# Jutho/Strided.jl

Hardware: AMD Instinct MI355X
Metric: GB/s effective HBM for @strided permutedims!+broadcast, 32^4 fp64 (higher is better)
Workload: dtype f64; 1 GPU; configs[1]+configs[2]: permutedims!(B,A,(4,3,2,1)) then C .= sum of 4 permuted views of A, 32x32x32x32 Float64, one set of arrays (A, B, C) per GPU.  C is a THIRD array chosen so that the two statements share only the read-only A and overlap; the README writes both into B -- that form is `step_same_destination` on the --full line; parallelism=replicas x1 (independent arrays per rank)

## Files before the change

include/strided_hip.h:

```cpp
#ifndef STRIDED_HIP_H
#define STRIDED_HIP_H

#include <stddef.h>
#include <stdint.h>

#ifdef __cplusplus
extern "C" {
#endif

#define SMR_ABI_VERSION 1
#define SMR_MAXN 8
#define SMR_MAXM 8
#define SMR_MAXPROG 96
#define SMR_MAXCONST 16

typedef enum {
    SMR_OK = 0,
    SMR_EINVAL = -1,
    SMR_EUNSUPPORTED = -2,
    SMR_EHIP = -3,
    SMR_ENOMEM = -4,
    SMR_ENODEVICE = -5
} smr_status;

// ... 106 lines not shown
    int64_t strides[SMR_MAXN];
    int32_t dtype;
    int32_t conj;
} smr_operand;

typedef struct smr_problem {
    int32_t N;
    int32_t M;
    int64_t dims[SMR_MAXN];
    smr_operand ops[SMR_MAXM];
    const uint8_t* fprog;
    int32_t fprog_len;
    int32_t nconsts;
    const double* fconsts;
    int32_t redop;
    int32_t initop;
    double initarg[2];
    void* stream;
} smr_problem;

typedef struct smr_plan smr_plan;

int smr_abi_version(void);
int smr_init(int device);
int smr_shutdown(void);
int smr_device_count(void);
const char* smr_last_error(void);
int smr_malloc(size_t bytes, void** out);
int smr_free(void* p);
int smr_memcpy_h2d(void* dst, const void* src, size_t bytes, void* stream);
int smr_memcpy_d2h(void* dst, const void* src, size_t bytes, void* stream);
int smr_stream_sync(void* stream);

int smr_overlap_begin(void* stream);
int smr_overlap_end(void* stream);
int smr_overlap_fence(void* stream);
int smr_stream_create(void** out);
int smr_stream_destroy(void* stream);

typedef struct smr_seq smr_seq;
int smr_seq_create(smr_seq** out);
int smr_seq_add(smr_seq* seq, smr_plan* plan, void* const* bases);
int smr_seq_run(smr_seq* seq, int reps, void* stream);
int smr_seq_wait(smr_seq* seq);
int smr_seq_info(smr_seq* seq, char* buf, size_t buflen);
int smr_seq_components(smr_seq* seq, int32_t* comp, size_t cap);
int smr_seq_fences(smr_seq* seq, int32_t* acquire, size_t cap, int64_t* footprint, int32_t* cache_resident);
int smr_seq_set(smr_seq* seq, const char* name, int64_t value);
int smr_seq_destroy(smr_seq* seq);
int smr_debug_kernarg_layout(const void* elf, size_t bytes, const char* symbol, int index, int32_t* out, char* name_out, size_t name_cap);
int smr_debug_canon_prog(const smr_problem* problem, uint8_t* code, int cap, int* nwraps, int* compute_class, int32_t* orig);
int smr_debug_seq_schedule(int nexec, const int32_t* nspans, const int64_t* spans, const int32_t* launches, const int64_t* knobs, const int32_t* comp_slices,
                           int32_t* per_exec, int32_t* totals, int64_t* footprint, int32_t* packets, int packet_cap);


int smr_mapreduce(const smr_problem* problem);
int smr_mapreduce_scalar(const smr_problem* problem, void* host_result);

int smr_plan_create(const smr_problem* problem, smr_plan** out);
int smr_plan_execute(smr_plan* plan, void* const* bases, void* stream);
int smr_plan_destroy(smr_plan* plan);
int smr_plan_prepare(smr_plan* plan);
int smr_plan_describe(const smr_plan* plan, char* buf, size_t buflen);
int64_t smr_plan_algorithmic_bytes(const smr_plan* plan);
int64_t smr_plan_tile_order(const smr_plan* plan, uint32_t* out, size_t cap);
int64_t smr_plan_orbit_pairs(const smr_plan* plan, uint32_t* out, size_t cap);
int64_t smr_plan_flat_runs(const smr_plan* plan, int64_t* out, size_t cap);
int64_t smr_plan_flat_side(const smr_plan* plan, int64_t* out, size_t cap);
int64_t smr_plan_flat_batched(const smr_plan* plan, int64_t* out, size_t cap);

int smr_plan_jit_compile(smr_plan* plan, size_t* code_size);
int smr_plan_jit_source(const smr_plan* plan, char* buf, size_t buflen);

int smr_shard(const smr_problem* problem, int nshards, int shard, smr_problem* out,
              int* needs_allreduce);
int smr_shard_ex(const smr_problem* problem, int nshards, int shard, uint32_t local_ops,
                 smr_problem* out, int* needs_allreduce, int* split_dim, int64_t* start,
                 int64_t* stop);
int smr_init_reduction(const smr_problem* problem);

int smr_comm_unique_id(void* out, size_t len);
int smr_comm_init(int nranks, int rank, const void* unique_id, size_t len);
int smr_comm_rank(int* rank, int* nranks);
int smr_comm_library(char* buf, size_t buflen);
int smr_comm_destroy(void);
int smr_mapreduce_sharded(const smr_problem* problem);
int smr_mapreduce_sharded_ex(const smr_problem* problem, uint32_t local_ops);

int smr_set_option(const char* name, int64_t value);
int64_t smr_get_option(const char* name);

#ifdef __cplusplus
}
#endif
#endif
```

strided.jl_amd/_lib.py:

```python
from __future__ import annotations

import ctypes as C
import os
import subprocess

SMR_MAXN = 8
SMR_MAXM = 8
SMR_MAXPROG = 96
SMR_MAXCONST = 16

SMR_OK, SMR_EINVAL, SMR_EUNSUPPORTED, SMR_EHIP, SMR_ENOMEM, SMR_ENODEVICE = 0, -1, -2, -3, -4, -5

(SMR_F32, SMR_F64, SMR_C32, SMR_C64, SMR_I8, SMR_I16, SMR_I32, SMR_I64,
 SMR_U8, SMR_U16, SMR_U32, SMR_U64, SMR_BOOL) = range(13)

SMR_RED_NONE, SMR_RED_ADD, SMR_RED_MUL, SMR_RED_MIN, SMR_RED_MAX, SMR_RED_AND, SMR_RED_OR = range(7)
(SMR_INIT_NONE, SMR_INIT_IDENTITY, SMR_INIT_ZERO, SMR_INIT_SCALE, SMR_INIT_CONST,
 SMR_INIT_CONJ) = range(6)

OPCODES = dict(
    ARG=0, CONST=1,
    NEG=8, ABS=9, ABS2=10, CONJ=11, REAL=12, IMAG=13, SQRT=14, EXP=15, LOG=16, SIN=17, COS=18,
    TANH=19, INV=20, ROUND32=21, WIDEN=22,
    ADD=32, SUB=33, MUL=34, DIV=35, MIN=36, MAX=37, LT=38, LE=39, GT=40, GE=41, EQ=42, NE=43,
    SELECT=64, FMA=65,
    POWI=96, TAN=97, ASIN=98, ACOS=99, ATAN=100, SINH=101, COSH=102, EXP2=103, EXPM1=104, LOG2=105, LOG10=106, LOG1P=107,
    CBRT=108, FLOOR=109, CEIL=110, TRUNC=111, ROUND=112, SIGN=113, NOT=114,
    POW=128, ATAN2=129, HYPOT=130, REM=131, MOD=132, AND=133, OR=134, XOR=135,
)


class smr_operand(C.Structure):
    _fields_ = [
        ("base", C.c_void_p),
        ("offset", C.c_int64),
        ("strides", C.c_int64 * SMR_MAXN),
        ("dtype", C.c_int32),
        ("conj", C.c_int32),
    ]


class smr_problem(C.Structure):
    _fields_ = [
        ("N", C.c_int32),
        ("M", C.c_int32),
        ("dims", C.c_int64 * SMR_MAXN),
        ("ops", smr_operand * SMR_MAXM),
        ("fprog", C.POINTER(C.c_uint8)),
        ("fprog_len", C.c_int32),
        ("nconsts", C.c_int32),
        ("fconsts", C.POINTER(C.c_double)),
        ("redop", C.c_int32),
        ("initop", C.c_int32),
        ("initarg", C.c_double * 2),
        ("stream", C.c_void_p),
    ]


_PKG_DIR = os.path.dirname(os.path.abspath(__file__))
LIB_PATH = os.environ.get("SMR_LIB") or os.path.join(_PKG_DIR, "libstrided_hip.so")
CSRC_DIR = os.path.join(_PKG_DIR, "csrc")

EXPORTS = [
    "smr_abi_version", "smr_init", "smr_shutdown", "smr_device_count", "smr_last_error",
    "smr_malloc", "smr_free", "smr_memcpy_h2d", "smr_memcpy_d2h", "smr_stream_sync",
    "smr_mapreduce", "smr_plan_create", "smr_plan_execute", "smr_plan_destroy",
    "smr_plan_describe", "smr_plan_algorithmic_bytes", "smr_plan_tile_order", "smr_plan_orbit_pairs", "smr_plan_flat_runs", "smr_plan_flat_side", "smr_plan_flat_batched", "smr_mapreduce_scalar", "smr_plan_jit_compile", "smr_plan_jit_source", "smr_plan_prepare", "smr_comm_unique_id", "smr_comm_init", "smr_comm_rank", "smr_comm_library",
    "smr_comm_destroy", "smr_mapreduce_sharded", "smr_mapreduce_sharded_ex", "smr_shard", "smr_shard_ex", "smr_init_reduction", "smr_set_option",
    "smr_get_option", "smr_overlap_begin", "smr_overlap_end", "smr_overlap_fence", "smr_stream_create", "smr_stream_destroy",
    "smr_seq_create", "smr_seq_add", "smr_seq_run", "smr_seq_wait", "smr_seq_info", "smr_seq_components", "smr_seq_fences", "smr_seq_set", "smr_seq_destroy", "smr_debug_kernarg_layout", "smr_debug_canon_prog", "smr_debug_seq_schedule",
]


class StridedHIPError(RuntimeError):
    def __init__(self, code, msg):
        super().__init__(f"libstrided_hip error {code}: {msg}")
        self.code = code


class UnsupportedOnDevice(StridedHIPError):
    """SMR_EUNSUPPORTED: valid in the reference but outside the device whitelist."""


def build(jobs: int | None = None, verbose: bool = False) -> str:
    if not jobs:
        try:
            jobs = int(os.environ.get("MAX_JOBS", "0"))
        except ValueError:
            jobs = 0
    jobs = jobs or min(16, len(os.sched_getaffinity(0)) if hasattr(os, "sched_getaffinity") else (os.cpu_count() or 1))
    jobs = max(1, jobs)
    r = subprocess.run(["make", "-C", CSRC_DIR, f"-j{jobs}"], capture_output=True, text=True)
    if r.returncode != 0:
        raise RuntimeError("building libstrided_hip.so failed:\n" + r.stdout[-4000:] + r.stderr[-8000:])
    if verbose:
        print(r.stdout[-2000:])
    return LIB_PATH


_lib = None


def load():
    global _lib
    if _lib is not None:
        return _lib
    if not os.path.exists(LIB_PATH):
        raise ImportError(
            f"{LIB_PATH} is missing: run `python -c 'import __graft_entry__ as g; g.build()'` "
            "(hipcc, gfx950).  strided_jl_amd has no CPU fallback.")
    try:
        import torch
    except Exception:
        pass
    lib = C.CDLL(LIB_PATH, mode=C.RTLD_GLOBAL)
    lib.smr_last_error.restype = C.c_char_p
    lib.smr_abi_version.restype = C.c_int
    lib.smr_init.argtypes = [C.c_int]
    lib.smr_malloc.argtypes = [C.c_size_t, C.POINTER(C.c_void_p)]
    lib.smr_free.argtypes = [C.c_void_p]
    lib.smr_memcpy_h2d.argtypes = [C.c_void_p, C.c_void_p, C.c_size_t, C.c_void_p]
    lib.smr_memcpy_d2h.argtypes = [C.c_void_p, C.c_void_p, C.c_size_t, C.c_void_p]
    lib.smr_stream_sync.argtypes = [C.c_void_p]
# ... 279 lines not shown
```

strided.jl_amd/csrc/smr_direct.cpp:

```cpp
#include <dlfcn.h>
#include <link.h>
#include <sched.h>
#include <sys/mman.h>
#include <unistd.h>

#include <algorithm>
#include <chrono>
#include <cstdio>
#include <cstdlib>
#include <cstring>

#include "smr_direct.h"

namespace smr {

static thread_local std::vector<RecLaunch>* tl_recorder = nullptr;
std::vector<RecLaunch>* recorder() { return tl_recorder; }
static thread_local bool tl_rec_seq = false, tl_self_released = false;
static thread_local bool tl_rec_eager = false;
void set_recorder(std::vector<RecLaunch>* r, bool allow_self_release, bool eager) {
    tl_recorder = r;
    tl_rec_seq = r != nullptr && allow_self_release;
    tl_rec_eager = r != nullptr && eager;
}
// ... 170 lines not shown
}

bool wait_signal(Direct& d, hsa_signal_t sig) {
    Hsa& h = hsa();
    if (h.signal_load(sig) == 0) return true;
    if (d.failed.load()) {
        direct_fail(d, "the HSA queue reported an error");
        return false;
    }
    double t0 = now_s();
    const double limit = direct_timeout_s();
    uint64_t seen[SEQ_MAXQ] = {};
    for (int k = 0; k < SEQ_MAXQ; ++k)
        if (d.q[k]) seen[k] = h.load_read_index(d.q[k]);
    for (;;) {
        if (h.signal_wait(sig, HSA_SIGNAL_CONDITION_EQ, 0, 200000, HSA_WAIT_STATE_ACTIVE) == 0) return true;
        if (d.failed.load()) {
            direct_fail(d, "the HSA queue reported an error");
            return false;
        }
        for (int k = 0; k < SEQ_MAXQ; ++k)
            if (d.q[k]) {
                const uint64_t r = h.load_read_index(d.q[k]);
                if (r != seen[k]) {
                    seen[k] = r;
                    t0 = now_s();
                }
            }
        if (now_s() - t0 > limit) {
            direct_fail(d, "no hardware queue made progress and the completion signal did not arrive within the time limit ($SMR_DIRECT_TIMEOUT_MS)");
            return false;
        }
    }
}

static std::mutex g_direct_mu;
static std::map<int, Direct*> g_direct;
std::vector<int> direct_devices() {
    std::lock_guard<std::mutex> g(g_direct_mu);
    std::vector<int> devs;
    for (auto& kv : g_direct) devs.push_back(kv.first);
    return devs;
}

int direct_queue(Direct& d, int k) {
    if (d.q[k]) return SMR_OK;
    Hsa& h = hsa();
    hsa_status_t st = h.queue_create(d.agent, 16384, HSA_QUEUE_TYPE_SINGLE, queue_error, &d, UINT32_MAX, UINT32_MAX, &d.q[k]);
    if (st != HSA_STATUS_SUCCESS) {
        d.q[k] = nullptr;
        d.why = "hsa_queue_create failed";
        return set_error(SMR_EHIP, d.why);
    }
    if (h.signal_create(0, 0, nullptr, &d.done[k]) != HSA_STATUS_SUCCESS) {
        d.why = "hsa_signal_create failed";
        return set_error(SMR_EHIP, d.why);
    }
    volatile hsa_signal_value_t* vp = nullptr;
    if (h.signal_value_pointer(d.done[k], &vp) == HSA_STATUS_SUCCESS) d.done_ptr[k] = (volatile int64_t*)vp;
    return SMR_OK;
}

int current_device() {
    int dev = 0;
    (void)hipGetDevice(&dev);
    return dev;
}
int device_of(hipStream_t s) {
    if (s) {
        hipDevice_t dv = 0;
        if (hipStreamGetDevice(s, &dv) == hipSuccess) return (int)dv;
        (void)hipGetLastError();
    }
    return current_device();
}

namespace {
int direct_selftest(Direct& d);
}

Direct& direct_of(int dev) {
    std::lock_guard<std::mutex> g(g_direct_mu);
    auto it = g_direct.find(dev);
    if (it != g_direct.end()) return *it->second;
    Direct* d = new Direct();
    d->dev = dev;
    g_direct[dev] = d;
    Hsa& h = hsa();
    if (!h.ok) {
        d->why = h.why;
        return *d;
    }
    hipDeviceProp_t prop;
    if (hipGetDeviceProperties(&prop, dev) != hipSuccess) {
        d->why = "hipGetDeviceProperties failed";
        return *d;
    }
    AgentPick pick;
    pick.h = &h;
    pick.bdf = ((uint32_t)prop.pciBusID << 8) | ((uint32_t)prop.pciDeviceID << 3);
    pick.domain = (uint32_t)prop.pciDomainID;
    h.iterate_agents(pick_agent, &pick);
    if (!pick.have) {
        if (pick.ngpu == 1) {
            pick.found = pick.first;
        } else {
            d->why = "no HSA agent matches the HIP device's PCI address";
            return *d;
        }
    }
    d->agent = pick.found;
// ... 246 lines not shown
        return done(SMR_EUNSUPPORTED, "hipHostMalloc failed");
    std::memset(out, 0, 64);
    KernelRef k;
    if (resolve_kernel(d, (const void*)k_direct_probe, k) != SMR_OK) return done(SMR_EUNSUPPORTED, smr_last_error());
    const unsigned grid = 5, block = 192, lds = 192 * 4, magic = 0x5eed0000u;
    std::vector<unsigned char> ex(12);
    std::memcpy(ex.data(), &out, 8);
    std::memcpy(ex.data() + 8, &magic, 4);
    KernargLayout lay;
    if (k.private_size != 0 || k.kernarg_size > 4096 || !kernarg_layout_of(k, ex.size(), lay)) return done(SMR_EUNSUPPORTED, "the probe kernel's arguments do not match its metadata");
    std::memset(kargs, 0, 4096);
    std::memcpy(kargs, ex.data(), ex.size());
    kmeta_fill_hidden(lay, (unsigned char*)kargs, grid, block, lds);
    hsa_kernel_dispatch_packet_t pk = dispatch_packet(k, grid, block, lds, kargs);
    pk.completion_signal = d.done[0];
    h.signal_store_relaxed(d.done[0], 1);
    if (!put_packet(d, d.q[0], &pk, header_of(true, HSA_FENCE_SCOPE_SYSTEM, HSA_FENCE_SCOPE_SYSTEM), pk.setup))
        return done(SMR_EUNSUPPORTED, "the probe packet could not be written (queue error)");
    const double t0 = now_s();
    while (h.signal_wait(d.done[0], HSA_SIGNAL_CONDITION_EQ, 0, 200000, HSA_WAIT_STATE_ACTIVE) != 0) {
        if (d.failed.load() || now_s() - t0 > std::min(5.0, direct_timeout_s())) {
            d.failed.store(true);
            {
                std::lock_guard<std::mutex> g(d.why_mu);
                d.fail_why = "the self-test packet did not complete";
            }
            out = nullptr;
            kargs = nullptr;
            return done(SMR_EUNSUPPORTED, "the probe packet did not complete (queue error or time-out)");
        }
    }
    const unsigned want2 = magic + block - 1;
    if (out[0] != block || out[1] != grid || out[2] != want2 || out[3] != grid) {
        char msg[200];
        std::snprintf(msg, sizeof msg, "the probe kernel saw blockDim %u (want %u), gridDim %u (want %u), LDS word 0x%x (want 0x%x), %u workgroups (want %u)", out[0], block,
                      out[1], grid, out[2], want2, out[3], grid);
        return done(SMR_EUNSUPPORTED, msg);
    }
    d.probe_ok = true;
    d.probe_meta = k.from_metadata;
    return done(SMR_OK, "");
}
}

const char* layout_source(const Direct& d) {
    if (!d.probe_ok) return d.n_meta > 0 && d.n_v5 == 0 ? "metadata" : "v5-rule(unverified)";
    if (d.n_v5 == 0) return "metadata+verified";
    return d.n_meta > 0 ? "metadata|v5-rule+verified" : "v5-rule+verified";
}

int wait_all(Direct& d) {
    bool any = false;
    int rc = SMR_OK;
    for (int k = 0; k < SEQ_MAXQ; ++k)
        if (d.armed[k]) {
            if (rc == SMR_OK && !wait_signal(d, d.done[k])) rc = SMR_EHIP;
            d.armed[k] = false;
            any = true;
        }
    if (any && rc == SMR_OK) d.last_us = (now_s() - d.t_submit) * 1e6;
    return rc;
}

}
```

strided.jl_amd/csrc/smr_sched.cpp:

```cpp
#include "smr_sched.h"

#include <algorithm>

namespace smr {

bool overlaps(const Spans& v, const std::pair<uintptr_t, uintptr_t>& x) {
    for (const auto& y : v)
        if (x.first < y.second && y.first < x.second) return true;
    return false;
}
bool overlaps(const Spans& v, const Spans& w) {
    for (const auto& x : w)
        if (overlaps(v, x)) return true;
    return false;
}

int components_of(const std::vector<Spans>& rd, const std::vector<Spans>& wr, std::vector<int>& comp) {
    const size_t ni = rd.size();
    std::vector<int> parent(ni);
    for (size_t i = 0; i < ni; ++i) parent[i] = (int)i;
    auto find = [&](int x) {
        while (parent[x] != x) x = parent[x] = parent[parent[x]];
        return x;
    };
// ... 157 lines not shown
                    unsigned lo = 0, hi = j == 0 ? ex[i].grid : 0;
                    if (ns > 1) slice_range(ex[i].grid, ns, s2, lo, hi);
                    if (j == 0 && hi <= lo) continue;
                    SchedEntry e;
                    e.exec = (int)i;
                    e.launch = j;
                    e.slice = s2;
                    e.lo = lo;
                    e.hi = hi;
                    e.barrier = j > 0 || !free_;
                    e.acquire = j > 0 || raw[i] != 0;
                    out.queues[k].push_back(e);
                }
            }
    }
}
}

Schedule schedule(const std::vector<SchedExec>& ex, const SchedKnobs& knobs) {
    Schedule out;
    const size_t ni = ex.size();
    out.footprint_bytes = union_bytes(ex);
    out.cache_resident = out.footprint_bytes <= knobs.self_release_max_total;
    Comps cs;
    {
        std::vector<Spans> rds(ni), wrs(ni);
        std::vector<size_t> bytes(ni, 0);
        for (size_t i = 0; i < ni; ++i) {
            rds[i] = ex[i].rd;
            wrs[i] = ex[i].wr;
            for (const auto& x : ex[i].rd) bytes[i] += x.second - x.first;
            for (const auto& x : ex[i].wr) bytes[i] += x.second - x.first;
        }
        out.ncomp = components_of(rds, wrs, out.comp);
        cs.first.assign(out.ncomp, -1);
        cs.bytes.assign(out.ncomp, 0);
        cs.slices.assign(out.ncomp, 1);
        cs.queue.assign(out.ncomp, 0);
        for (size_t i = 0; i < ni; ++i) {
            cs.bytes[out.comp[i]] += bytes[i];
            if (cs.first[out.comp[i]] < 0) cs.first[out.comp[i]] = (int)i;
        }
    }
    const int maxq = std::max(1, knobs.max_queues);
    out.nsliced = choose_slices(ex, knobs, out.comp, maxq, cs);
    out.nq = assign_queues(maxq, cs);
    out.queue.resize(ni);
    out.nslices.resize(ni);
    for (size_t i = 0; i < ni; ++i) {
        out.queue[i] = cs.queue[out.comp[i]];
        out.nslices[i] = cs.slices[out.comp[i]];
    }
    order_packets(ex, knobs, cs, out);
    return out;
}

}
```

strided.jl_amd/csrc/smr_sched.h:

```cpp
#pragma once
#include <cstdint>
#include <map>
#include <utility>
#include <vector>

namespace smr {

typedef std::vector<std::pair<uintptr_t, uintptr_t>> Spans;
bool overlaps(const Spans& v, const std::pair<uintptr_t, uintptr_t>& x);
bool overlaps(const Spans& v, const Spans& w);

struct SchedExec {
    Spans rd, wr;
    int nlaunch = 0;
    unsigned grid = 0;
    bool sliceable = false;
    bool all_self = false;
    int same_as = 0;
};
struct SchedKnobs {
    int max_queues = 4;
    int slices = -1;
    std::map<int, int> comp_slices;
    bool all_ordered = false;
    int64_t self_release_max_total = 0;
};
struct SchedEntry {
    int exec, launch, slice;
    unsigned lo, hi;
    bool barrier, acquire;
};
struct Schedule {
    std::vector<int> comp, acquire, queue, nslices;
    int ncomp = 0, nsliced = 0, nq = 0;
    int64_t footprint_bytes = 0;
    bool cache_resident = false;
    std::vector<std::vector<SchedEntry>> queues;
};

int components_of(const std::vector<Spans>& rd, const std::vector<Spans>& wr, std::vector<int>& comp);
void slice_range(unsigned grid, int ns, int s, unsigned& lo, unsigned& hi);
Schedule schedule(const std::vector<SchedExec>& ex, const SchedKnobs& knobs);

}
```

strided.jl_amd/csrc/smr_seq.cpp:

```cpp
#include <sched.h>

#include <algorithm>
#include <cstdio>
#include <cstdlib>
#include <cstring>

#include "smr_direct.h"

using namespace smr;

struct SeqItem {
    smr_plan* plan;
    bool has_bases;
    void* bases[SMR_MAXM];
};
struct SeqPacket {
    hsa_kernel_dispatch_packet_t pk;
    bool barrier;
    bool acquire;
    bool self_released;
};
struct smr_seq {
    std::vector<SeqItem> items;
    bool built = false;
    bool aql = false;
    std::string why_not_aql;
    std::vector<SeqPacket> packets[SEQ_MAXQ];
    int nq = 0;
    int max_queues = 4;
    int slices = -1;
    std::map<int, int> comp_slices;
    int nsliced = 0;
    int ncomp = 0;
    void* d_kernargs = nullptr;
    std::vector<std::shared_ptr<void>> keep;
    int64_t runs = 0;
    int n_any = 0, n_barrier = 0, n_acquire = 0, n_self_released = 0;
    int acq_mid = -1, rel_mid = 1;
    int rel_self = 0;
    int acq_first = -1, rel_last = 2;
    int acq_first_auto = 2;
    bool all_ordered = false;
    bool inflight = false;
    int device = -1;
    int async_mode = -1;
    bool held = false;
};


namespace {
__global__ void k_seq_hold(const volatile long long* const* sigs, int n, unsigned long long limit, unsigned* gave_up) {
    if (threadIdx.x != 0) return;
    const unsigned long long t0 = wall_clock64();
    for (int k = 0; k < n; ++k)
        while (__hip_atomic_load((const long long*)sigs[k], __ATOMIC_RELAXED, __HIP_MEMORY_SCOPE_SYSTEM) != 0) {
            __builtin_amdgcn_s_sleep(64);
            if (wall_clock64() - t0 > limit) {
                __hip_atomic_store(gave_up, 1u, __ATOMIC_RELAXED, __HIP_MEMORY_SCOPE_SYSTEM);
                return;
            }
        }
}

struct Rec {
    std::vector<RecLaunch> launches;
    std::vector<KernelRef> refs;
    std::vector<size_t> offs;
    size_t blocksize(size_t j) const { return (std::max<size_t>(refs[j].kernarg_size, launches[j].args.size()) + 255) & ~(size_t)255; }
};
void* const* bases_of(const SeqItem& it) { return it.has_bases ? it.bases : nullptr; }

std::vector<SchedExec> seq_footprints(smr_seq* q) {
    std::vector<SchedExec> ex(q->items.size());
    for (size_t i = 0; i < ex.size(); ++i) {
        const SeqItem& it = q->items[i];
        seq_footprint(it.plan, bases_of(it), ex[i].rd, ex[i].wr);
        ex[i].same_as = (int)i;
        for (size_t j = 0; j < i && ex[i].same_as == (int)i; ++j) {
            const SeqItem& o = q->items[j];
            if (o.plan == it.plan && o.has_bases == it.has_bases && !(it.has_bases && std::memcmp(it.bases, o.bases, sizeof it.bases) != 0)) ex[i].same_as = (int)j;
        }
    }
    return ex;
}
SchedKnobs seq_knobs(const smr_seq* q) {
    SchedKnobs k;
    k.max_queues = std::max(1, std::min(q->max_queues, SEQ_MAXQ));
    k.slices = q->slices;
    k.comp_slices = q->comp_slices;
    k.all_ordered = q->all_ordered;
    k.self_release_max_total = options().self_release_max_total;
    return k;
}

int seq_record(smr_seq* q, std::vector<Rec>& recs, std::vector<SchedExec>& ex) {
    for (const SeqItem& it : q->items)
        if (int rc = seq_execute_plan(it.plan, bases_of(it), nullptr, true)) return rc;
    ex = seq_footprints(q);
    const bool allow_self = schedule(ex, seq_knobs(q)).cache_resident;
    for (size_t i = 0; i < q->items.size(); ++i) {
        set_recorder(&recs[i].launches, allow_self);
        int rc = seq_execute_plan(q->items[i].plan, bases_of(q->items[i]), nullptr, false);
        set_recorder(nullptr);
        if (rc) return rc;
        if (recs[i].launches.empty()) return set_error(SMR_EINVAL, "smr_seq: a plan recorded no launch");
        const RecLaunch& l0 = recs[i].launches[0];
        ex[i].nlaunch = (int)recs[i].launches.size();
        ex[i].grid = l0.grid;
        ex[i].sliceable = l0.slice_kind != 0;
        ex[i].all_self = true;
        for (const RecLaunch& l : recs[i].launches) ex[i].all_self = ex[i].all_self && l.self_released;
    }
    return SMR_OK;
}

bool seq_resolve(smr_seq* q, Direct& d, std::vector<Rec>& recs) {
    for (Rec& r : recs)
        for (const RecLaunch& l : r.launches) {
            if (l.keep) q->keep.push_back(l.keep);
            KernelRef k;
            if (!resolve_launch(d, l, k, &q->why_not_aql)) return false;
            r.refs.push_back(k);
        }
    return true;
}

int seq_kernargs(smr_seq* q, std::vector<Rec>& recs, const Schedule& sc) {
    size_t total = 0;
    for (size_t i = 0; i < recs.size(); ++i)
        for (size_t j = 0; j < recs[i].launches.size(); ++j) {
            recs[i].offs.push_back(total);
            total += recs[i].blocksize(j) * (size_t)sc.nslices[i];
        }
    std::vector<unsigned char> host(total, 0);
    for (size_t i = 0; i < recs.size(); ++i)
        for (size_t j = 0; j < recs[i].launches.size(); ++j) {
            const RecLaunch& l = recs[i].launches[j];
            const int ns = sc.nslices[i];
            for (int s2 = 0; s2 < ns; ++s2) {
                unsigned lo = 0, hi = l.grid;
                if (ns > 1) slice_range(l.grid, ns, s2, lo, hi);
                unsigned char* b = host.data() + recs[i].offs[j] + (size_t)s2 * recs[i].blocksize(j);
                fill_kernarg_image(recs[i].refs[j], l, hi - lo, b, recs[i].blocksize(j));
                if (ns > 1 && l.slice_kind == 1) {
                    uint32_t v;
                    std::memcpy(&v, b + l.slice_off, 4);
                    v += lo;
                    std::memcpy(b + l.slice_off, &v, 4);
                } else if (ns > 1 && l.slice_kind == 2) {
                    uint64_t v;
                    std::memcpy(&v, b + l.slice_off, 8);
                    v += (uint64_t)lo * l.slice_row;
                    std::memcpy(b + l.slice_off, &v, 8);
                }
#if SMR_STAMP
                if (ns > 1 && l.args.size() >= 8) {
                    uint64_t sp = 0;
                    std::memcpy(&sp, b + l.args.size() - 8, 8);
                    if (sp) {
                        sp += (uint64_t)lo * ((l.block + 63) / 64) * 16;
                        std::memcpy(b + l.args.size() - 8, &sp, 8);
                    }
                }
#endif
            }
        }
    if (q->d_kernargs) (void)hipFree(q->d_kernargs);
    q->d_kernargs = nullptr;
    hipError_t e = hipMalloc(&q->d_kernargs, total ? total : 256);
    if (e != hipSuccess) return hip_error(e, "hipMalloc(sequence kernargs)");
    e = hipMemcpy(q->d_kernargs, host.data(), total, hipMemcpyHostToDevice);
    if (e != hipSuccess) return hip_error(e, "hipMemcpy(sequence kernargs)");
    return SMR_OK;
}

int seq_first_acquire_scope(const std::vector<SchedExec>& ex, int device) {
    for (const SchedExec& r : ex)
        for (const auto& x : r.rd) {
            hipPointerAttribute_t at;
            std::memset(&at, 0, sizeof at);
            const bool local = x.second > x.first && hipPointerGetAttributes(&at, (const void*)x.first) == hipSuccess && at.type == hipMemoryTypeDevice &&
                               !at.isManaged && at.device == device;
            if (!local) {
                (void)hipGetLastError();
                return HSA_FENCE_SCOPE_SYSTEM;
            }
        }
    return HSA_FENCE_SCOPE_AGENT;
}

int seq_build(smr_seq* q) {
    for (auto& v : q->packets) v.clear();
    q->keep.clear();
    q->aql = false;
    q->n_any = q->n_barrier = q->n_acquire = q->n_self_released = 0;
    q->nq = 0;
    q->nsliced = 0;
    q->device = current_device();
    Direct& d = direct_of(q->device);
    if (!d.ok) {
        std::lock_guard<std::mutex> g(d.why_mu);
        q->why_not_aql = d.why;
    }
    std::vector<Rec> recs(q->items.size());
    std::vector<SchedExec> ex;
    if (int rc = seq_record(q, recs, ex)) return rc;
    std::unique_lock<std::mutex> dlock(d.mu);
    const bool aql = d.ok && seq_resolve(q, d, recs);
    dlock.unlock();
    q->aql = aql;
    q->built = true;
    if (!aql) return SMR_OK;
    const Schedule sc = schedule(ex, seq_knobs(q));
    q->ncomp = sc.ncomp;
    q->nsliced = sc.nsliced;
    dlock.lock();
    for (int k = 0; k < sc.nq; ++k)
        if (int rc = direct_queue(d, k)) return rc;
    dlock.unlock();
    q->nq = sc.nq;
    if (int rc = seq_kernargs(q, recs, sc)) return rc;
    q->acq_first_auto = seq_first_acquire_scope(ex, q->device);
    for (int k = 0; k < sc.nq; ++k)
        for (const SchedEntry& e : sc.queues[k]) {
            const Rec& r = recs[e.exec];
            const RecLaunch& l = r.launches[e.launch];
            const unsigned nblocks = sc.nslices[e.exec] > 1 ? e.hi - e.lo : l.grid;
            if (nblocks == 0) continue;
            SeqPacket sp;
            std::memset(&sp, 0, sizeof sp);
            sp.barrier = e.barrier;
            sp.acquire = e.acquire;
            sp.self_released = l.self_released;
            if (sp.self_released) ++q->n_self_released;
            (sp.barrier ? q->n_barrier : q->n_any)++;
            if (sp.acquire) ++q->n_acquire;
            sp.pk = dispatch_packet(r.refs[e.launch], nblocks, l.block, l.lds, (char*)q->d_kernargs + r.offs[e.launch] + (size_t)e.slice * r.blocksize(e.launch));
            q->packets[k].push_back(sp);
        }
    return SMR_OK;
}

int seq_submit(smr_seq* q, Direct& d, int reps) {
    Hsa& h = hsa();
    const int acq_mid = q->acq_mid, rel_mid = q->rel_mid;
    uint64_t written[SEQ_MAXQ] = {}, totalp[SEQ_MAXQ] = {};
    int open_queues = 0;
    for (int k = 0; k < q->nq; ++k) {
        totalp[k] = (uint64_t)q->packets[k].size() * (uint64_t)reps;
        d.armed[k] = totalp[k] > 0;
        if (totalp[k]) {
            h.signal_store_relaxed(d.done[k], 1);
            ++open_queues;
        }
    }
    d.t_submit = now_s();
    double t_progress = d.t_submit;
    unsigned idle_rounds = 0;
    while (open_queues > 0) {
        if (++idle_rounds > 64) {
            if (idle_rounds < 1024) __builtin_ia32_pause();
            else sched_yield();
            if ((idle_rounds & 1023) == 0 && (d.failed.load() || now_s() - t_progress > direct_timeout_s())) {
                direct_fail(d, "the hardware queues stopped consuming packets during a replay");
                return SMR_EHIP;
            }
        }
        for (int k = 0; k < q->nq; ++k) {
            if (written[k] >= totalp[k]) continue;
            hsa_queue_t* hq = d.q[k];
            const uint32_t mask = hq->size - 1;
            const size_t np = q->packets[k].size();
            const uint64_t widx = h.add_write_index(hq, 0);
            const uint64_t room = hq->size - (widx - h.load_read_index(hq));
            if (room == 0) continue;
            const uint64_t nthis = std::min<uint64_t>({room, totalp[k] - written[k], (uint64_t)256});
            const uint64_t base = h.add_write_index(hq, nthis);
            for (uint64_t t = 0; t < nthis; ++t) {
                const uint64_t g = written[k] + t;
                const SeqPacket& sp = q->packets[k][g % np];
                hsa_kernel_dispatch_packet_t* slot = (hsa_kernel_dispatch_packet_t*)hq->base_address + ((base + t) & mask);
                const bool first = g == 0, last = g + 1 == totalp[k];
                hsa_kernel_dispatch_packet_t pk = sp.pk;
                pk.completion_signal = last ? d.done[k] : hsa_signal_t{0};
                std::memcpy((char*)slot + 4, (const char*)&pk + 4, sizeof pk - 4);
                const int acq = acq_mid >= 0 ? acq_mid : (sp.acquire ? HSA_FENCE_SCOPE_AGENT : HSA_FENCE_SCOPE_NONE);
                const int rel = (sp.self_released && q->rel_self == 0) ? HSA_FENCE_SCOPE_NONE : rel_mid;
                const uint16_t hdr = header_of(sp.barrier || first, first ? (q->acq_first >= 0 ? q->acq_first : q->acq_first_auto) : acq, last ? q->rel_last : rel);
                __atomic_store_n((uint32_t*)slot, (uint32_t)hdr | ((uint32_t)pk.setup << 16), __ATOMIC_RELEASE);
            }
            h.signal_store_screlease(hq->doorbell_signal, (hsa_signal_value_t)(base + nthis - 1));
            idle_rounds = 0;
            t_progress = now_s();
            written[k] += nthis;
            if (written[k] >= totalp[k]) --open_queues;
        }
    }
    return SMR_OK;
}

struct HoldBlock {
    const volatile long long** sigs = nullptr;
    unsigned* gave_up = nullptr;
};
HoldBlock* hold_block(Direct& d) {
    static std::mutex mu;
    static std::map<int, HoldBlock> all;
    std::lock_guard<std::mutex> g(mu);
    HoldBlock& hb = all[d.dev];
    if (!hb.sigs) {
        void* p = nullptr;
        if (hipHostMalloc(&p, 256, hipHostMallocDefault) != hipSuccess) {
            (void)hipGetLastError();
            return nullptr;
        }
        std::memset(p, 0, 256);
        hb.sigs = (const volatile long long**)p;
        hb.gave_up = (unsigned*)((char*)p + 128);
    }
    return &hb;
}
}

extern "C" {

int smr_seq_create(smr_seq** out) {
    if (!out) return set_error(SMR_EINVAL, "null out");
    *out = new (std::nothrow) smr_seq();
    return *out ? SMR_OK : set_error(SMR_ENOMEM, "out of host memory");
}

int smr_seq_add(smr_seq* q, smr_plan* plan, void* const* bases) {
    if (!q || !plan) return set_error(SMR_EINVAL, "null argument");
    if (q->inflight) return set_error(SMR_EINVAL, "smr_seq_add: a replay is in flight (smr_seq_wait first)");
    SeqItem it;
    std::memset(&it, 0, sizeof it);
    it.plan = plan;
    it.has_bases = bases != nullptr;
    if (bases)
        for (int k = 0; k < seq_nops(plan); ++k) it.bases[k] = bases[k];
    q->items.push_back(it);
// ... 58 lines not shown
    HoldBlock* hb = hold_block(d);
    int n = 0;
    if (hb)
        for (int k = 0; k < q->nq; ++k)
            if (d.armed[k] && d.done_ptr[k]) hb->sigs[n++] = (const volatile long long*)d.done_ptr[k];
    bool all_have_ptr = hb != nullptr;
    for (int k = 0; k < q->nq; ++k)
        if (d.armed[k] && !d.done_ptr[k]) all_have_ptr = false;
    if (all_have_ptr && n > 0) {
        (void)hipGetLastError();
        const unsigned long long limit = (unsigned long long)(std::max(direct_timeout_s() * 20.0, 600.0) * 1e8);
        hipLaunchKernelGGL(k_seq_hold, dim3(1), dim3(64), 0, s, (const volatile long long* const*)hb->sigs, n, limit, hb->gave_up);
        if (hipGetLastError() == hipSuccess) {
            q->held = true;
            return SMR_OK;
        }
    }
    rc = wait_all(d);
    q->inflight = false;
    return rc;
}

int smr_seq_wait(smr_seq* q) {
    if (!q) return set_error(SMR_EINVAL, "null sequence");
    if (!q->aql || !q->inflight) return SMR_OK;
    Direct& d = direct_of(q->device);
    int rc;
    {
        std::lock_guard<std::mutex> g(d.mu);
        rc = wait_all(d);
    }
    q->inflight = false;
    if (rc == SMR_OK && q->held) {
        HoldBlock* hb = hold_block(d);
        if (hb && __atomic_load_n(hb->gave_up, __ATOMIC_RELAXED)) {
            __atomic_store_n(hb->gave_up, 0u, __ATOMIC_RELAXED);
            rc = set_error(SMR_EHIP, "smr_seq: the holding kernel on the caller's stream gave up before the replay completed");
        }
    }
    return rc;
}

int smr_seq_info(smr_seq* q, char* buf, size_t buflen) {
    if (!q || !buf || !buflen) return set_error(SMR_EINVAL, "null argument");
    if (!q->built) {
        int rc = seq_build(q);
        if (rc) return rc;
    }
    if (q->aql) {
        const Direct& d = direct_of(q->device);
        size_t np = 0;
        for (const auto& v : q->packets) np += v.size();
        const int first = q->acq_first >= 0 ? q->acq_first : q->acq_first_auto;
        std::snprintf(buf, buflen, "backend=aql items=%zu packets=%zu components=%d sliced=%d queues=%d ordered=%d unordered=%d acquire=%s(%d of %zu packets) first_acquire=%s release=%d self_released=%d kernarg_layout=%s agent=%s stream_wait=%s last_replay_us=%.3f",
                      q->items.size(), np, q->ncomp, q->nsliced, q->nq, q->n_barrier, q->n_any, q->acq_mid < 0 ? "by-need" : (q->acq_mid == 0 ? "none" : (q->acq_mid == 1 ? "agent" : "system")),
                      q->n_acquire, np, first == 2 ? "system" : (first == 1 ? "agent" : "none"), q->rel_mid, q->n_self_released, layout_source(d), d.agent_by_pci ? "pci-address" : "only-gpu",
                      q->async_mode == 0 ? "host(blocking)" : (d.wait_value_ok ? "hipStreamWaitValue64" : "holding-kernel|owned-stream"), d.last_us);
    }
    else
        std::snprintf(buf, buflen, "backend=hip items=%zu (%s)", q->items.size(), q->why_not_aql.c_str());
    return SMR_OK;
}

int smr_seq_components(smr_seq* q, int32_t* comp, size_t cap) {
    if (!q) return set_error(SMR_EINVAL, "null sequence");
    const Schedule sc = schedule(seq_footprints(q), seq_knobs(q));
    if (comp)
        for (size_t i = 0; i < sc.comp.size() && i < cap; ++i) comp[i] = sc.comp[i];
    return sc.ncomp;
}

int smr_seq_fences(smr_seq* q, int32_t* acquire, size_t cap, int64_t* footprint, int32_t* cache_resident) {
    if (!q) return set_error(SMR_EINVAL, "null sequence");
    const Schedule sc = schedule(seq_footprints(q), seq_knobs(q));
    if (acquire)
        for (size_t i = 0; i < sc.acquire.size() && i < cap; ++i) acquire[i] = sc.acquire[i];
    if (footprint) *footprint = sc.footprint_bytes;
    if (cache_resident) *cache_resident = sc.cache_resident ? 1 : 0;
    return (int)sc.acquire.size();
}

int smr_debug_seq_schedule(int nexec, const int32_t* nspans, const int64_t* spans, const int32_t* launches, const int64_t* knobs, const int32_t* comp_slices,
                           int32_t* per_exec, int32_t* totals, int64_t* footprint, int32_t* packets, int packet_cap) {
    if (nexec < 0 || !nspans || !spans || !launches || !knobs) return set_error(SMR_EINVAL, "smr_debug_seq_schedule: null argument");
    std::vector<SchedExec> ex((size_t)nexec);
    for (int i = 0; i < nexec; ++i) {
        for (int k = 0; k < nspans[2 * i] + nspans[2 * i + 1]; ++k, spans += 2)
            (k < nspans[2 * i] ? ex[i].rd : ex[i].wr).push_back({(uintptr_t)spans[0], (uintptr_t)spans[1]});
        const int32_t* l = launches + 5 * i;
        ex[i].nlaunch = l[0];
        ex[i].grid = (unsigned)l[1];
        ex[i].sliceable = l[2] != 0;
        ex[i].all_self = l[3] != 0;
        ex[i].same_as = l[4];
    }
    SchedKnobs kn;
    kn.max_queues = (int)knobs[0];
    kn.slices = (int)knobs[1];
    kn.all_ordered = knobs[2] != 0;
    kn.self_release_max_total = knobs[3];
    for (int64_t c = 0; comp_slices && c < knobs[4]; ++c) kn.comp_slices[comp_slices[2 * c]] = comp_slices[2 * c + 1];
    const Schedule sc = schedule(ex, kn);
    for (int i = 0; per_exec && i < nexec; ++i) {
        const int32_t row[4] = {sc.comp[i], sc.acquire[i], sc.queue[i], sc.nslices[i]};
        std::memcpy(per_exec + 4 * i, row, sizeof row);
    }
    if (totals) {
        totals[0] = sc.ncomp;
        totals[1] = sc.nsliced;
        totals[2] = sc.nq;
        totals[3] = sc.cache_resident ? 1 : 0;
    }
    if (footprint) *footprint = sc.footprint_bytes;
    int n = 0;
    for (int k = 0; k < sc.nq; ++k)
        for (const SchedEntry& e : sc.queues[k]) {
            if (packets && n < packet_cap) {
                const int32_t row[8] = {k, e.exec, e.launch, e.slice, (int32_t)e.lo, (int32_t)e.hi, e.barrier ? 1 : 0, e.acquire ? 1 : 0};
                std::memcpy(packets + 8 * n, row, sizeof row);
            }
            ++n;
        }
    return n;
}

int smr_seq_set(smr_seq* q, const char* name, int64_t value) {
    if (!q || !name) return set_error(SMR_EINVAL, "null argument");
    static const struct {
        const char* name;
        int smr_seq::*member;
        int lo, hi;
        bool rebuilds;
    } table[] = {
        {"acquire", &smr_seq::acq_mid, -1, 2, false},
        {"release", &smr_seq::rel_mid, 0, 2, false},
        {"release_self", &smr_seq::rel_self, 0, 1, false},
        {"first_acquire", &smr_seq::acq_first, -1, 2, false},
        {"last_release", &smr_seq::rel_last, 0, 2, false},
        {"async", &smr_seq::async_mode, -1, 1, false},
        {"queues", &smr_seq::max_queues, 1, SEQ_MAXQ, true},
    };
    if (std::strcmp(name, "fence_scope") == 0 && value >= 0 && value <= 2) {
        q->acq_mid = q->rel_mid = (int)value;
        return SMR_OK;
    }
    for (const auto& t : table)
        if (std::strcmp(name, t.name) == 0 && value >= t.lo && value <= t.hi && !(t.rebuilds && q->inflight)) {
            q->*t.member = (int)value;
            if (t.rebuilds) q->built = false;
            return SMR_OK;
        }
    if (q->inflight) return set_error(SMR_EINVAL, "smr_seq_set: a replay is in flight (smr_seq_wait first)");
    if (std::strcmp(name, "order") == 0) {
        q->all_ordered = value == 0;
        q->built = false;
        return SMR_OK;
    }
    if (std::strcmp(name, "slices") == 0 && (value == -1 || (value >= 1 && value <= SEQ_MAXQ))) {
        q->slices = (int)value;
        q->comp_slices.clear();
        q->built = false;
        return SMR_OK;
    }
    if (std::strncmp(name, "slices:", 7) == 0 && value >= 1 && value <= SEQ_MAXQ) {
        char* end = nullptr;
        const long c = std::strtol(name + 7, &end, 10);
        if (end == name + 7 || *end || c < 0 || c > 4096) return set_error(SMR_EINVAL, "smr_seq_set: slices:<component>");
        q->comp_slices[(int)c] = (int)value;
        q->built = false;
        return SMR_OK;
    }
    return set_error(SMR_EINVAL, "smr_seq_set: unknown name");
}

int smr_seq_destroy(smr_seq* q) {
    if (!q) return SMR_OK;
    (void)smr_seq_wait(q);
    if (q->d_kernargs) (void)hipFree(q->d_kernargs);
    delete q;
    return SMR_OK;
}

}
```

Before: 7868 GB/s.

## Auto-pick last-packet release scope, use GPU-only completion signals, skip idle waits

Measured after the change: 7816 GB/s. About the same (-0.7%).

```diff
diff --git a/include/strided_hip.h b/include/strided_hip.h
--- a/include/strided_hip.h
+++ b/include/strided_hip.h
@@ -182,6 +182,9 @@
 int smr_debug_canon_prog(const smr_problem* problem, uint8_t* code, int cap, int* nwraps, int* compute_class, int32_t* orig);
 int smr_debug_seq_schedule(int nexec, const int32_t* nspans, const int64_t* spans, const int32_t* launches, const int64_t* knobs, const int32_t* comp_slices,
                            int32_t* per_exec, int32_t* totals, int64_t* footprint, int32_t* packets, int packet_cap);
+int smr_debug_seq_schedule_release(int nexec, const int32_t* nspans, const int64_t* spans, const int32_t* launches, const int64_t* knobs, const int32_t* comp_slices,
+                                   int32_t* per_exec, int32_t* totals, int64_t* footprint, int32_t* packets, int packet_cap, const int32_t* wr_local,
+                                   int last_release, int32_t* release, int release_cap);
 
 
 int smr_mapreduce(const smr_problem* problem);
diff --git a/strided.jl_amd/_lib.py b/strided.jl_amd/_lib.py
--- a/strided.jl_amd/_lib.py
+++ b/strided.jl_amd/_lib.py
@@ -68,7 +68,7 @@
     "smr_plan_describe", "smr_plan_algorithmic_bytes", "smr_plan_tile_order", "smr_plan_orbit_pairs", "smr_plan_flat_runs", "smr_plan_flat_side", "smr_plan_flat_batched", "smr_mapreduce_scalar", "smr_plan_jit_compile", "smr_plan_jit_source", "smr_plan_prepare", "smr_comm_unique_id", "smr_comm_init", "smr_comm_rank", "smr_comm_library",
     "smr_comm_destroy", "smr_mapreduce_sharded", "smr_mapreduce_sharded_ex", "smr_shard", "smr_shard_ex", "smr_init_reduction", "smr_set_option",
     "smr_get_option", "smr_overlap_begin", "smr_overlap_end", "smr_overlap_fence", "smr_stream_create", "smr_stream_destroy",
-    "smr_seq_create", "smr_seq_add", "smr_seq_run", "smr_seq_wait", "smr_seq_info", "smr_seq_components", "smr_seq_fences", "smr_seq_set", "smr_seq_destroy", "smr_debug_kernarg_layout", "smr_debug_canon_prog", "smr_debug_seq_schedule",
+    "smr_seq_create", "smr_seq_add", "smr_seq_run", "smr_seq_wait", "smr_seq_info", "smr_seq_components", "smr_seq_fences", "smr_seq_set", "smr_seq_destroy", "smr_debug_kernarg_layout", "smr_debug_canon_prog", "smr_debug_seq_schedule", "smr_debug_seq_schedule_release",
 ]
 
 
diff --git a/strided.jl_amd/csrc/smr_direct.cpp b/strided.jl_amd/csrc/smr_direct.cpp
--- a/strided.jl_amd/csrc/smr_direct.cpp
+++ b/strided.jl_amd/csrc/smr_direct.cpp
@@ -246,11 +246,21 @@
         d.why = "hsa_queue_create failed";
         return set_error(SMR_EHIP, d.why);
     }
+    const char* sg = std::getenv("SMR_EAGER_SIGNALS");
+    volatile hsa_signal_value_t* vp = nullptr;
+    if (h.amd_signal_create && !(sg && std::strcmp(sg, "interrupt") == 0) &&
+        h.amd_signal_create(0, 0, nullptr, HSA_AMD_SIGNAL_AMD_GPU_ONLY, &d.done[k]) == HSA_STATUS_SUCCESS) {
+        if (h.signal_value_pointer(d.done[k], &vp) == HSA_STATUS_SUCCESS) {
+            d.done_ptr[k] = (volatile int64_t*)vp;
+            return SMR_OK;
+        }
+        (void)h.signal_destroy(d.done[k]);
+        d.done[k] = hsa_signal_t{0};
+    }
     if (h.signal_create(0, 0, nullptr, &d.done[k]) != HSA_STATUS_SUCCESS) {
         d.why = "hsa_signal_create failed";
         return set_error(SMR_EHIP, d.why);
     }
-    volatile hsa_signal_value_t* vp = nullptr;
     if (h.signal_value_pointer(d.done[k], &vp) == HSA_STATUS_SUCCESS) d.done_ptr[k] = (volatile int64_t*)vp;
     return SMR_OK;
 }
@@ -603,11 +613,16 @@
 int wait_all(Direct& d) {
     bool any = false;
     int rc = SMR_OK;
+    bool pending = false;
     for (int k = 0; k < SEQ_MAXQ; ++k)
         if (d.armed[k]) {
-            if (rc == SMR_OK && !wait_signal(d, d.done[k])) rc = SMR_EHIP;
+            any = true;
+            pending = pending || hsa().signal_load(d.done[k]) != 0;
+        }
+    for (int k = 0; k < SEQ_MAXQ; ++k)
+        if (d.armed[k]) {
+            if (pending && rc == SMR_OK && !wait_signal(d, d.done[k])) rc = SMR_EHIP;
             d.armed[k] = false;
-            any = true;
         }
     if (any && rc == SMR_OK) d.last_us = (now_s() - d.t_submit) * 1e6;
     return rc;
diff --git a/strided.jl_amd/csrc/smr_sched.cpp b/strided.jl_amd/csrc/smr_sched.cpp
--- a/strided.jl_amd/csrc/smr_sched.cpp
+++ b/strided.jl_amd/csrc/smr_sched.cpp
@@ -233,6 +233,15 @@
         out.nslices[i] = cs.slices[out.comp[i]];
     }
     order_packets(ex, knobs, cs, out);
+    bool all_local = true;
+    for (const SchedExec& r : ex) all_local = all_local && r.wr_local;
+    out.last_release_set = knobs.last_release >= 0;
+    out.last_release.assign(out.nq, 2);
+    for (int k = 0; k < out.nq; ++k) {
+        bool queue_self = all_local;
+        for (const SchedEntry& e : out.queues[k]) queue_self = queue_self && ex[e.exec].all_self;
+        out.last_release[k] = out.last_release_set ? knobs.last_release : (queue_self ? 0 : 2);
+    }
     return out;
 }
 
diff --git a/strided.jl_amd/csrc/smr_sched.h b/strided.jl_amd/csrc/smr_sched.h
--- a/strided.jl_amd/csrc/smr_sched.h
+++ b/strided.jl_amd/csrc/smr_sched.h
@@ -16,6 +16,7 @@
     unsigned grid = 0;
     bool sliceable = false;
     bool all_self = false;
+    bool wr_local = false;
     int same_as = 0;
 };
 struct SchedKnobs {
@@ -24,6 +25,7 @@
     std::map<int, int> comp_slices;
     bool all_ordered = false;
     int64_t self_release_max_total = 0;
+    int last_release = -1;
 };
 struct SchedEntry {
     int exec, launch, slice;
@@ -36,6 +38,8 @@
     int64_t footprint_bytes = 0;
     bool cache_resident = false;
     std::vector<std::vector<SchedEntry>> queues;
+    std::vector<int> last_release;
+    bool last_release_set = false;
 };
 
 int components_of(const std::vector<Spans>& rd, const std::vector<Spans>& wr, std::vector<int>& comp);
diff --git a/strided.jl_amd/csrc/smr_seq.cpp b/strided.jl_amd/csrc/smr_seq.cpp
--- a/strided.jl_amd/csrc/smr_seq.cpp
+++ b/strided.jl_amd/csrc/smr_seq.cpp
@@ -38,8 +38,9 @@
     int n_any = 0, n_barrier = 0, n_acquire = 0, n_self_released = 0;
     int acq_mid = -1, rel_mid = 1;
     int rel_self = 0;
-    int acq_first = -1, rel_last = 2;
+    int acq_first = -1, rel_last = -1;
     int acq_first_auto = 2;
+    int rel_last_auto[SEQ_MAXQ] = {};
     bool all_ordered = false;
     bool inflight = false;
     int device = -1;
@@ -91,6 +92,20 @@
     k.all_ordered = q->all_ordered;
     k.self_release_max_total = options().self_release_max_total;
     return k;
+}
+
+bool all_local(const Spans& spans, int device) {
+    for (const auto& x : spans) {
+        hipPointerAttribute_t at;
+        std::memset(&at, 0, sizeof at);
+        const bool local = x.second > x.first && hipPointerGetAttributes(&at, (const void*)x.first) == hipSuccess && at.type == hipMemoryTypeDevice &&
+                           !at.isManaged && at.device == device;
+        if (!local) {
+            (void)hipGetLastError();
+            return false;
+        }
+    }
+    return true;
 }
 
 int seq_record(smr_seq* q, std::vector<Rec>& recs, std::vector<SchedExec>& ex) {
@@ -110,6 +125,7 @@
         ex[i].sliceable = l0.slice_kind != 0;
         ex[i].all_self = true;
         for (const RecLaunch& l : recs[i].launches) ex[i].all_self = ex[i].all_self && l.self_released;
+        ex[i].wr_local = all_local(ex[i].wr, q->device);
     }
     return SMR_OK;
 }
@@ -176,16 +192,7 @@
 
 int seq_first_acquire_scope(const std::vector<SchedExec>& ex, int device) {
     for (const SchedExec& r : ex)
-        for (const auto& x : r.rd) {
-            hipPointerAttribute_t at;
-            std::memset(&at, 0, sizeof at);
-            const bool local = x.second > x.first && hipPointerGetAttributes(&at, (const void*)x.first) == hipSuccess && at.type == hipMemoryTypeDevice &&
-                               !at.isManaged && at.device == device;
-            if (!local) {
-                (void)hipGetLastError();
-                return HSA_FENCE_SCOPE_SYSTEM;
-            }
-        }
+        if (!all_local(r.rd, device)) return HSA_FENCE_SCOPE_SYSTEM;
     return HSA_FENCE_SCOPE_AGENT;
 }
 
@@ -221,6 +228,7 @@
     q->nq = sc.nq;
     if (int rc = seq_kernargs(q, recs, sc)) return rc;
     q->acq_first_auto = seq_first_acquire_scope(ex, q->device);
+    for (int k = 0; k < sc.nq; ++k) q->rel_last_auto[k] = sc.last_release[k];
     for (int k = 0; k < sc.nq; ++k)
         for (const SchedEntry& e : sc.queues[k]) {
             const Rec& r = recs[e.exec];
@@ -271,10 +279,12 @@
             hsa_queue_t* hq = d.q[k];
             const uint32_t mask = hq->size - 1;
             const size_t np = q->packets[k].size();
+            const int rel_last = q->rel_last >= 0 ? q->rel_last : q->rel_last_auto[k];
             const uint64_t widx = h.add_write_index(hq, 0);
             const uint64_t room = hq->size - (widx - h.load_read_index(hq));
             if (room == 0) continue;
-            const uint64_t nthis = std::min<uint64_t>({room, totalp[k] - written[k], (uint64_t)256});
+            const uint64_t visit = written[k] == 0 ? std::min<uint64_t>(np, 256) : 256;
+            const uint64_t nthis = std::min<uint64_t>({room, totalp[k] - written[k], visit});
             const uint64_t base = h.add_write_index(hq, nthis);
             for (uint64_t t = 0; t < nthis; ++t) {
                 const uint64_t g = written[k] + t;
@@ -286,7 +296,7 @@
                 std::memcpy((char*)slot + 4, (const char*)&pk + 4, sizeof pk - 4);
                 const int acq = acq_mid >= 0 ? acq_mid : (sp.acquire ? HSA_FENCE_SCOPE_AGENT : HSA_FENCE_SCOPE_NONE);
                 const int rel = (sp.self_released && q->rel_self == 0) ? HSA_FENCE_SCOPE_NONE : rel_mid;
-                const uint16_t hdr = header_of(sp.barrier || first, first ? (q->acq_first >= 0 ? q->acq_first : q->acq_first_auto) : acq, last ? q->rel_last : rel);
+                const uint16_t hdr = header_of(sp.barrier || first, first ? (q->acq_first >= 0 ? q->acq_first : q->acq_first_auto) : acq, last ? rel_last : rel);
                 __atomic_store_n((uint32_t*)slot, (uint32_t)hdr | ((uint32_t)pk.setup << 16), __ATOMIC_RELEASE);
             }
             h.signal_store_screlease(hq->doorbell_signal, (hsa_signal_value_t)(base + nthis - 1));
@@ -451,10 +461,13 @@
         size_t np = 0;
         for (const auto& v : q->packets) np += v.size();
         const int first = q->acq_first >= 0 ? q->acq_first : q->acq_first_auto;
-        std::snprintf(buf, buflen, "backend=aql items=%zu packets=%zu components=%d sliced=%d queues=%d ordered=%d unordered=%d acquire=%s(%d of %zu packets) first_acquire=%s release=%d self_released=%d kernarg_layout=%s agent=%s stream_wait=%s last_replay_us=%.3f",
+        int last = q->rel_last;
+        for (int k = 0; k < q->nq && q->rel_last < 0; ++k) last = std::max(last, q->rel_last_auto[k]);
+        std::snprintf(buf, buflen, "backend=aql items=%zu packets=%zu components=%d sliced=%d queues=%d ordered=%d unordered=%d acquire=%s(%d of %zu packets) first_acquire=%s release=%d self_released=%d kernarg_layout=%s agent=%s stream_wait=%s last_release=%s(%s) last_replay_us=%.3f",
                       q->items.size(), np, q->ncomp, q->nsliced, q->nq, q->n_barrier, q->n_any, q->acq_mid < 0 ? "by-need" : (q->acq_mid == 0 ? "none" : (q->acq_mid == 1 ? "agent" : "system")),
                       q->n_acquire, np, first == 2 ? "system" : (first == 1 ? "agent" : "none"), q->rel_mid, q->n_self_released, layout_source(d), d.agent_by_pci ? "pci-address" : "only-gpu",
-                      q->async_mode == 0 ? "host(blocking)" : (d.wait_value_ok ? "hipStreamWaitValue64" : "holding-kernel|owned-stream"), d.last_us);
+                      q->async_mode == 0 ? "host(blocking)" : (d.wait_value_ok ? "hipStreamWaitValue64" : "holding-kernel|owned-stream"),
+                      last == 2 ? "system" : (last == 1 ? "agent" : "none"), q->rel_last >= 0 ? "set" : "auto", d.last_us);
     }
     else
         std::snprintf(buf, buflen, "backend=hip items=%zu (%s)", q->items.size(), q->why_not_aql.c_str());
@@ -479,9 +492,11 @@
     return (int)sc.acquire.size();
 }
 
-int smr_debug_seq_schedule(int nexec, const int32_t* nspans, const int64_t* spans, const int32_t* launches, const int64_t* knobs, const int32_t* comp_slices,
-                           int32_t* per_exec, int32_t* totals, int64_t* footprint, int32_t* packets, int packet_cap) {
+int smr_debug_seq_schedule_release(int nexec, const int32_t* nspans, const int64_t* spans, const int32_t* launches, const int64_t* knobs, const int32_t* comp_slices,
+                                   int32_t* per_exec, int32_t* totals, int64_t* footprint, int32_t* packets, int packet_cap, const int32_t* wr_local,
+                                   int last_release, int32_t* release, int release_cap) {
     if (nexec < 0 || !nspans || !spans || !launches || !knobs) return set_error(SMR_EINVAL, "smr_debug_seq_schedule: null argument");
+    if (last_release < -1 || last_release > 2) return set_error(SMR_EINVAL, "smr_debug_seq_schedule_release: last_release is -1..2");
     std::vector<SchedExec> ex((size_t)nexec);
     for (int i = 0; i < nexec; ++i) {
         for (int k = 0; k < nspans[2 * i] + nspans[2 * i + 1]; ++k, spans += 2)
@@ -492,12 +507,14 @@
         ex[i].sliceable = l[2] != 0;
         ex[i].all_self = l[3] != 0;
         ex[i].same_as = l[4];
+        ex[i].wr_local = wr_local && wr_local[i] != 0;
     }
     SchedKnobs kn;
     kn.max_queues = (int)knobs[0];
     kn.slices = (int)knobs[1];
     kn.all_ordered = knobs[2] != 0;
     kn.self_release_max_total = knobs[3];
+    kn.last_release = last_release;
     for (int64_t c = 0; comp_slices && c < knobs[4]; ++c) kn.comp_slices[comp_slices[2 * c]] = comp_slices[2 * c + 1];
     const Schedule sc = schedule(ex, kn);
     for (int i = 0; per_exec && i < nexec; ++i) {
@@ -511,6 +528,10 @@
         totals[3] = sc.cache_resident ? 1 : 0;
     }
     if (footprint) *footprint = sc.footprint_bytes;
+    for (int k = 0; release && k < sc.nq && k < release_cap; ++k) {
+        release[2 * k] = sc.last_release[k];
+        release[2 * k + 1] = sc.last_release_set ? 1 : 0;
+    }
     int n = 0;
     for (int k = 0; k < sc.nq; ++k)
         for (const SchedEntry& e : sc.queues[k]) {
@@ -521,6 +542,10 @@
             ++n;
         }
     return n;
+}
+int smr_debug_seq_schedule(int nexec, const int32_t* nspans, const int64_t* spans, const int32_t* launches, const int64_t* knobs, const int32_t* comp_slices,
+                           int32_t* per_exec, int32_t* totals, int64_t* footprint, int32_t* packets, int packet_cap) {
+    return smr_debug_seq_schedule_release(nexec, nspans, spans, launches, knobs, comp_slices, per_exec, totals, footprint, packets, packet_cap, nullptr, -1, nullptr, 0);
 }
 
 int smr_seq_set(smr_seq* q, const char* name, int64_t value) {
@@ -535,7 +560,7 @@
         {"release", &smr_seq::rel_mid, 0, 2, false},
         {"release_self", &smr_seq::rel_self, 0, 1, false},
         {"first_acquire", &smr_seq::acq_first, -1, 2, false},
-        {"last_release", &smr_seq::rel_last, 0, 2, false},
+        {"last_release", &smr_seq::rel_last, -1, 2, false},
         {"async", &smr_seq::async_mode, -1, 1, false},
         {"queues", &smr_seq::max_queues, 1, SEQ_MAXQ, true},
     };
```
